# nygenome/lancet

Measured on AMD Instinct MI355X. Metric: assembled windows/sec (whole node), 600bp windows, self-tuning k, synthetic T/N, higher is better.
Workload: dtype u64; 1 GPU; chr22-scan proxy: 32768 windows/GPU x 600 bp, stride 100, 30x tumor / 30x normal, 2x150 bp, k=11..101, active-region-off; windows_per_gpu=32768, reads_per_gpu=5895305, records_rank0_contig=22477, slots_in_flight=4080, batches_in_flight=2, windows_first_graph_in_lds=32768, graphs_built_ahead=2147, graphs_taken_from_pool=2037, windows_rerun_worst_case_tier=0

## Files before the change

lancet_amd/csrc/kernels.h:

```cpp
#pragma once
#include "wave.h"
#include "layout.h"
#include "../../include/lancet_engine.h"

#ifndef LANCET_WG
#define LANCET_WG 64
#endif
#ifdef LANCET_FAT
#define LC_QLANES LC_FAT_LANES
#define LC_PF_G 6
#define LC_QSTAGE (3 * LC_FAT_LANES)
#else
#define LC_QLANES LANCET_WG
#define LC_QSTAGE LC_STAGE
#endif

enum {
  EV_PROCESS = 1, EV_REPEAT_REF, EV_NEAR_REF, EV_READS, EV_STATS, EV_MARKREF, EV_LOWCOV, EV_CLEANDEAD,
  EV_COMPRESS, EV_CC, EV_CCID, EV_CCEND, EV_TRIM, EV_AMBIG_SRC, EV_NOMATCH_SRC, EV_AMBIG_SNK, EV_NOMATCH_SNK,
  EV_CYCLE, EV_TIPS_ROUND, EV_TIPS_REMOVED, EV_LINKS, EV_LOOKREP, EV_MISSING, EV_SEARCH, EV_NEAR_QRY,
  EV_DFSLIMIT, EV_PATH, EV_TS, EV_PATH_END, EV_EKA_END, EV_FOUND, EV_END
};

struct WinShared {
// ... 4159 lines not shown
  for (int j = 0; j < 3; ++j) {
    if (r.nh[j] < t.hrmnN[j]) t.hrmnN[j] = r.nh[j];
    if (r.th[j] < t.hrmnT[j]) t.hrmnT[j] = r.th[j];
    t.hrsumN[j] = (uint16_t)(t.hrsumN[j] + r.nh[j]); t.hrsumT[j] = (uint16_t)(t.hrsumT[j] + r.th[j]);
  }
}
DEV void ref_hp_at(const Ctx &c, uint32_t pos, HPc &r) {
  for (int j = 0; j < 3; ++j) { r.nh[j] = r.th[j] = r.nq[j] = r.tq[j] = 0; }
  if (!LC_SREF(c).LR || (int)pos >= LC_SREF(c).reflen) return;
  const uint16_t *h = LC_CTX(c).W->refhp + 6 * pos;
  for (int j = 0; j < 3; ++j) { r.th[j] = h[j]; r.nh[j] = h[3 + j]; }
}
DEV void path_hp_at(const Ctx &c, int P, HPc &a) {
  for (int j = 0; j < 3; ++j) { a.nh[j] = a.th[j] = a.nq[j] = a.tq[j] = 0; }
  if (!LC_SREF(c).LR) return;
  uint32_t d = LC_CTX(c).W->pdesc[P];
  desc_hp(c, d, 0, a.nh, a.nq);
  desc_hp(c, d, 1, a.th, a.tq);
}
template <class T> DEV void ts_add_alt(T &t, const uint16_t *n4, const uint16_t *t4) { for (int q = 0; q < 4; ++q) { acc_push(t.aN[q], n4[q]); acc_push(t.aT[q], t4[q]); } }
template <class T> DEV void ts_add_ref(T &t, const uint16_t *n2, const uint16_t *t2) { for (int q = 0; q < 2; ++q) { acc_push(t.rN[q], n2[q]); acc_push(t.rT[q], t2[q]); } }

DEV void ref_cov_at(const Ctx &c, uint32_t pos, uint16_t *n2, uint16_t *t2) {
  if ((int)pos < LC_SREF(c).reflen) { const uint16_t *r = LC_CTX(c).W->refcov + 4 * pos; t2[0] = r[0]; t2[1] = r[1]; n2[0] = r[2]; n2[1] = r[3]; }
  else { n2[0] = n2[1] = t2[0] = t2[1] = 0; }
}
DEV void path_cov_at(const Ctx &c, int P, uint16_t *n4, uint16_t *t4) {
  uint32_t d = LC_CTX(c).W->pdesc[P];
  desc_cov(c, d, 0, &n4[0], &n4[1], &n4[2], &n4[3]);
  desc_cov(c, d, 1, &t4[0], &t4[1], &t4[2], &t4[3]);
}

DEV void bx_add_node(Ctx &c, uint32_t X, uint32_t nml, uint32_t *n) {
  LC_GLOBAL Work &W = *LC_CTX(c).W; LC_GLOBAL const DevBatch &B = *LC_CTX(c).B; LC_WS &S = LC_SREF(c);
  const uint32_t g0 = B.read_begin[S.w], refr = (uint32_t)(S.R - 1);
  LC_GLOBAL uint32_t *buf = W.bxbuf;
  for (uint32_t i = W.nocc[X]; i < W.nocc[X + 1]; ++i) {
    const uint32_t r = CS_READ(W_CSR(W)[i]);
    if (r == refr) continue;
    if (RI_NML(B.rinfo[g0 + r]) != nml) continue;
    const uint32_t bx = B.bx_rank[g0 + r];
    if (bx == 0xFFFFFFFFu) continue;
    uint32_t lo = 0, hi = *n;
    while (lo < hi) { uint32_t mid = (lo + hi) >> 1; if (buf[mid] < bx) lo = mid + 1; else hi = mid; }
    if (lo < *n && buf[lo] == bx) continue;
    if (*n >= LC_CTX(c).C->reads_cap) { OVF(c); return; }
    for (uint32_t j = *n; j > lo; --j) buf[j] = buf[j - 1];
    buf[lo] = bx; ++*n;
  }
}
DEVNI uint32_t kmer_lookup(Ctx &c, const uint8_t *codes, int *ori) {
  LC_GLOBAL Work &W = *LC_CTX(c).W; LC_WS &S = LC_SREF(c);
  const int K = S.K, NW = S.NW;
  unsigned long long fw[LC_NWMAX], rc[LC_NWMAX];
  for (int w = 0; w < LC_NWMAX; ++w) { fw[w] = 0; rc[w] = 0; }
  for (int i = 0; i < K; ++i) { key_push_fw(fw, NW, K, codes[i] & 3); key_push_rc(rc, NW, K, codes[i] & 3); }
  const unsigned long long *ck = key_less(fw, rc, NW) ? fw : rc;
  if (ori) *ori = ck == fw ? 0 : (key_less(rc, fw, NW) ? 1 : 2);
  const uint32_t mask = S.tmask;
  unsigned long long h = 0; uint32_t idx;
  if (NW == 1 && K <= 31) { h = ck[0] + 1ULL; idx = (uint32_t)mix64(h) & mask; }
  else {
    for (int w = 0; w < NW; ++w) h = mix64(h ^ (ck[w] + 0x9e3779b97f4a7c15ULL * (unsigned long long)(w + 1)));
    h &= ~(1ULL << 63);
    if (h == 0) h = 1;
    idx = (uint32_t)h & mask;
  }
  for (uint32_t probes = 0; probes <= mask; ++probes) {
    const unsigned long long cur = SL_TAG(W, idx);
    if (cur == 0) return LC_NIL;
    if (cur == h) {
      bool same = true;
      if (!(NW == 1 && K <= 31)) for (int w = 0; w < NW; ++w) if (W.slot_key[(size_t)idx * LC_NWMAX + w] != ck[w]) same = false;
      if (same) return SL_NODE(W, idx);
    }
    idx = (idx + 1) & mask;
  }
  return LC_NIL;
}
DEVNI void emit_variant_lr(Ctx &c, uint32_t vi, const TS &t, const uint16_t hp12[12], int plen) {
  LC_WS &S = LC_SREF(c); LC_GLOBAL Work &W = *LC_CTX(c).W; DevOut &O = *LC_CTX(c).OUT;
  lancet_variant_lr &l = O.variants_lr[vi];
  for (int q = 0; q < 12; ++q) l.hp[q] = hp12[q];
  l.reserved[0] = l.reserved[1] = 0;
  const int K = S.K;
  const uint32_t ro = W.occ_base[S.R - 1];
  for (int q = 0; q < 4; ++q) {
    const uint32_t nml = (q == 0 || q == 2) ? 1u : 0u;
    uint32_t n = 0;
    if (q < 2) {
      for (int i = (int)t.ref_pos - 1; i <= (int)t.ref_end_pos - 1; ++i) {
        if (i < 0 || i + K > S.seq_len) continue;
        const uint32_t rv = S.prebuilt ? W.lr_refnode[S.seq_t5 + i] : 0u;
        const uint32_t X = S.prebuilt ? (rv & 0x3FFFFFFFu) : (W.occ[ro + (uint32_t)(S.seq_t5 + i)] & 0x3FFFFFFFu);
        if (S.prebuilt ? (rv >> 31) != 0u : (W.gr[X].flags & NF_INMER) != 0u) bx_add_node(c, X, nml, &n);
      }
    } else {
      for (int i = (int)t.start_pos - 2; i <= (int)t.end_pos - 1; ++i) {
        if (i < 0 || i + K > plen) continue;
        const uint32_t X = kmer_lookup(c, W.pseq + i);
        if (X != LC_NIL) bx_add_node(c, X, nml, &n);
      }
    }
    const uint32_t off = dev_atomic_add(O.n_bx, n);
    if (off + n > LC_CTX(c).C->bx_cap) { OVF(c); l.bx_off[q] = 0; l.bx_len[q] = 0; continue; }
    l.bx_off[q] = off; l.bx_len[q] = n;
    for (uint32_t j = 0; j < n; ++j) O.bx_blob[off + j] = W.bxbuf[j];
  }
}

DEVNI void emit_variant(Ctx &c, const TS &t, const uint16_t cov[8], int strLen, const uint8_t *motif, int motifLen, bool hasStr,
                      const uint8_t *ra, const uint8_t *pa, const uint16_t hp12[12], int plen) {
  LC_WS &S = LC_SREF(c); DevOut &O = *LC_CTX(c).OUT;
  uint32_t vi = dev_atomic_add(O.n_variants, 1u);
  int rl = t.col1 - t.col0 + 1;
  char sbuf[80]; int sl = 0;
  if (hasStr) {
    char digs[12]; int nd = 0; int v = strLen; do { digs[nd++] = (char)('0' + v % 10); v /= 10; } while (v);
    while (nd) sbuf[sl++] = digs[--nd];
    for (int i = 0; i < motifLen; ++i) sbuf[sl++] = "ACGT"[motif[i]];
  }
  uint32_t need = (uint32_t)(2 * rl + sl);
  uint32_t bo = dev_atomic_add(O.n_blob, need);
  if (vi >= LC_CTX(c).C->var_cap || bo + need > LC_CTX(c).C->blob_cap) { OVF(c); return; }
  lancet_variant &v = O.variants[vi];
  v.window = S.w; v.seq_in_window = S.emit_seq++; v.chr_id = LC_CTX(c).B->chr_id[S.w]; v.pos = (int32_t)t.pos - 1;
  v.code = (uint8_t)t.code; v.prev_bp_ref = (uint8_t)t.prev_bp_ref; v.prev_bp_alt = (uint8_t)t.prev_bp_alt; v.reserved = 0;
  v.kmer = (uint16_t)S.K; for (int q = 0; q < 8; ++q) v.cov[q] = cov[q]; v.reserved2 = 0;
  v.ref_off = bo; v.ref_len = (uint32_t)rl; v.alt_off = bo + (uint32_t)rl; v.alt_len = (uint32_t)rl; v.str_off = bo + 2u * (uint32_t)rl; v.str_len = (uint32_t)sl;
  for (int i = 0; i < rl; ++i) { O.blob[bo + i] = (char)ra[t.col0 + i]; O.blob[bo + rl + i] = (char)pa[t.col0 + i]; }
  for (int i = 0; i < sl; ++i) O.blob[bo + 2 * rl + i] = sbuf[i];
  if (S.LR) emit_variant_lr(c, vi, t, hp12, plen);
}

DEVNI void walk_prepare(Ctx &c, int L) {
  LC_WS &S = LC_SREF(c); LC_GLOBAL Work &W = *LC_CTX(c).W;
  const int cap = (int)LC_CTX(c).C->max_w + (int)LC_CTX(c).C->path_cap + 2;
  LC_GLOBAL const uint8_t *ra = W.aln, *pa = W.aln + cap;
  LC_GLOBAL uint32_t *E1 = W.scratch, *E2 = W.scratch + (L + 1), *F = W.scratch + 2 * (L + 1), *cols = W.scratch + 3 * (L + 1);
  WG_LANE0 { S.wk[0] = S.wk[1] = S.wk[2] = S.wk[3] = 0; E1[L] = 0; E2[L] = 0; F[L] = 0; }
  WG_FOR(i, L) {
    const uint8_t r = ra[i], p = pa[i];
    E1[i] = r != '-'; E2[i] = p != '-'; F[i] = r != p;
    const int t = r == p ? 0 : (r == '-' ? 2 : (p == '-' ? 3 : 1));
    dev_atomic_add((LC_LDS uint32_t *)&S.wk[t], 1u);
  }
  WG_SYNC();
  wg_scan(E1, L + 1, S, S.part2);
  wg_scan(E2, L + 1, S, S.part2);
  wg_scan(F, L + 1, S, S.part2);
  WG_FOR(i, L) { if (F[i + 1] != F[i]) cols[F[i]] = (uint32_t)i; }
  WG_LANE0 { S.wk_n = (int)F[L]; }
}

DEVNI void process_path_walk(Ctx &c, int np, int plen, int L, int complete) {
  LC_WS &S = LC_SREF(c); LC_GLOBAL Work &W = *LC_CTX(c).W;
  const int K = S.K;
  const int cap = (int)LC_CTX(c).C->max_w + (int)LC_CTX(c).C->path_cap + 2;
  LC_GLOBAL const uint8_t *ra = W.aln, *pa = W.aln + cap;
  const int refstart = LC_CTX(c).B->ref_start[S.w];
  TS *ts = (TS *)(void *)W.tb;
  auto ts_at = [&](int idx) -> TS & { return ts[idx]; };
  int nts = 0;
  unsigned pos_in_ref = 0, pathpos = 0;
  char code = '?', prev_code = '?';
  const int match_bp = S.wk[0], snp_bp = S.wk[1], ins_bp = S.wk[2], del_bp = S.wk[3];
  LC_GLOBAL const uint32_t *E1 = W.scratch, *E2 = W.scratch + (L + 1), *cols = W.scratch + 3 * (L + 1);
  int pc_i = 0, pc_cur = 0;
  int last_col = -2;
  for (int ci = 0; ci < S.wk_n; ++ci) {
    const int i = (int)cols[ci];
    prev_code = (last_col == i - 1) ? code : '=';
    last_col = i;
    if (ra[i] == '-') code = '^'; else if (pa[i] == '-') code = 'v'; else code = 'x';
    pos_in_ref = E1[i];
    pathpos = E2[i] + (pa[i] != '-' ? 1u : 0u);
    uint32_t spanner = LC_NIL;
    for (; pc_i < np; ++pc_i) {
      const uint32_t nd = W.pnodes[pc_i];
      if (W.gr[nd].flags & NF_SPECIAL) continue;
      const int span = n_len(c, nd);
      if (pc_cur + span >= (int)pathpos) { spanner = nd; break; }
      pc_cur += span - K + 1;
    }
    if (spanner == LC_NIL) break;
    bool within_tumor = status_cnt_T(c, spanner);
    int P = (int)pathpos - 1;
    if (P < 0 || P >= plen) { OVF(c); return; }
    {
      uint16_t cn4[4], ct4[4], rn2[2], rt2[2];
      path_cov_at(c, P, cn4, ct4);
      ref_cov_at(c, pos_in_ref + (uint32_t)S.trim5, rn2, rt2);
      HPc ha, hr;
      path_hp_at(c, P, ha);
      ref_hp_at(c, pos_in_ref + (uint32_t)S.trim5, hr);
      unsigned rrpos = pos_in_ref + (unsigned)refstart + (unsigned)S.trim5;
      int pr = i - 1, pq = i - 1;
      while (pr >= 0 && ra[pr] != 'A' && ra[pr] != 'C' && ra[pr] != 'G' && ra[pr] != 'T') --pr;
      while (pq >= 0 && pa[pq] != 'A' && pa[pq] != 'C' && pa[pq] != 'G' && pa[pq] != 'T') --pq;
      if (pr < 0 || pq < 0) { OVF(c); return; }
      if (nts > 0 && prev_code != '=') {
        TS &t = ts_at(nts - 1);
        if (within_tumor) t.somatic = true;
        int reflen_before = t.col1 - t.col0 + 1;
        t.col1 = i; t.end_pos = (uint32_t)P; t.ref_end_pos = pos_in_ref;
        if (code == '^' && t.code == code && t.pos == rrpos) { ts_add_alt(t, cn4, ct4); ts_hp_add_alt(t, ha); }
        else if (code == 'v' && t.code == code && (t.pos + (unsigned)(reflen_before + 1)) == rrpos) { ts_add_ref(t, rn2, rt2); ts_hp_add_ref(t, hr); }
        else if (code == 'x' || t.code != code) { t.code = 'c'; ts_add_alt(t, cn4, ct4); ts_add_ref(t, rn2, rt2); ts_hp_add_alt(t, ha); ts_hp_add_ref(t, hr); }
      } else {
        if (nts >= LC_MAXTS) { OVF(c); return; }
        TS &t = ts_at(nts++);
        t.pos = rrpos; t.ref_pos = pos_in_ref; t.start_pos = (uint32_t)(P + 1); t.code = code; t.end_pos = (uint32_t)P; t.ref_end_pos = pos_in_ref;
        t.col0 = i; t.col1 = i; t.somatic = within_tumor; t.prev_bp_ref = (char)ra[pr]; t.prev_bp_alt = (char)pa[pq];
        for (int q = 0; q < 4; ++q) { acc_init(t.aN[q], cn4[q]); acc_init(t.aT[q], ct4[q]); }
        for (int q = 0; q < 2; ++q) { acc_init(t.rN[q], rn2[q]); acc_init(t.rT[q], rt2[q]); }
        ts_hp_init(t, ha, hr);
      }
    }
  }
  evt(c, EV_PATH, (uint32_t)complete, (uint32_t)S.tmp3, (uint32_t)match_bp, (uint32_t)snp_bp, (uint32_t)ins_bp, (uint32_t)del_bp);
  int ct_i = 0, ct_cur = 0, ct_last = -1;
  auto contig_at = [&](int pos) -> uint32_t {
    if (pos < ct_last) { ct_i = 0; ct_cur = 0; }
    ct_last = pos;
    for (; ct_i < np; ++ct_i) {
      const uint32_t nd = W.pnodes[ct_i];
      if (W.gr[nd].flags & NF_SPECIAL) continue;
      const int span = n_len(c, nd);
      if (ct_cur + span >= pos) return nd;
      ct_cur += span - K + 1;
    }
    return LC_NIL;
  };
  for (int ti = 0; ti < nts; ++ti) {
    TS &t = ts_at(ti);
    if (t.code != 'x') {
      for (int j = 0; j <= K; ++j) {
        unsigned idx1 = t.end_pos + (unsigned)j;
        if (idx1 < (unsigned)plen) {
          uint32_t sp = contig_at((int)idx1);
          if (sp == LC_NIL) break;
          if (status_cnt_T(c, sp)) t.somatic = true;
          uint16_t cn4[4], ct4[4];
          path_cov_at(c, (int)idx1, cn4, ct4);
          ts_add_alt(t, cn4, ct4);
          if (S.LR) { HPc ha; path_hp_at(c, (int)idx1, ha); ts_hp_add_alt(t, ha); }
        }
        unsigned idx2 = t.ref_end_pos + (unsigned)S.trim5 + (unsigned)j;
        uint16_t rn2[2], rt2[2];
        ref_cov_at(c, idx2, rn2, rt2);
        ts_add_ref(t, rn2, rt2);
        if (S.LR) { HPc hr; ref_hp_at(c, idx2, hr); ts_hp_add_ref(t, hr); }
      }
    }
    bool x = t.code == 'x';
    uint16_t RCNF = t.rN[0].mn, RCNR = t.rN[1].mn, RCTF = t.rT[0].mn, RCTR = t.rT[1].mn;
    uint16_t ACNF = x ? t.aN[2].mn : t.aN[0].mn, ACNR = x ? t.aN[3].mn : t.aN[1].mn;
    if (!x) { ACNF = t.aN[0].mnz; ACNR = t.aN[1].mnz; }
    uint16_t ACTF = x ? t.aT[2].mn : t.aT[0].mn, ACTR = x ? t.aT[3].mn : t.aT[1].mn;
    if (t.somatic) { RCNF = acc_mean(t.rN[0]); RCNR = acc_mean(t.rN[1]); RCTF = acc_mean(t.rT[0]); RCTR = acc_mean(t.rT[1]); ACNF = 0; ACNR = 0; }
    uint16_t cov[8] = {RCNF, RCNR, RCTF, RCTR, ACNF, ACNR, ACTF, ACTR};
    uint16_t hp12[12];
    {
      const uint32_t nref = t.rN[0].n;
      auto mean = [&](uint16_t sum) -> uint16_t { return nref > 0 ? (uint16_t)((float)sum / (float)nref) : (uint16_t)0; };
      uint16_t RN[3], RT[3], AN[3], AT[3];
      for (int j = 0; j < 3; ++j) {
        RN[j] = t.hrmnN[j]; RT[j] = t.hrmnT[j];
        AN[j] = x ? t.haqN[j] : t.hamnN[j]; AT[j] = x ? t.haqT[j] : t.hamnT[j];
        if (t.somatic) { RT[j] = mean(t.hrsumT[j]); RN[j] = mean(t.hrsumN[j]); AN[j] = 0; }
        if (!S.LR) { RN[j] = RT[j] = AN[j] = AT[j] = 0; }
      }
      const uint16_t v[12] = {RN[1], RN[2], RN[0], RT[1], RT[2], RT[0], AN[1], AN[2], AN[0], AT[1], AT[2], AT[0]};
      for (int q = 0; q < 12; ++q) hp12[q] = v[q];
    }
    if (LC_CTX(c).C->evt_cap) {
      evt(c, EV_TS, t.pos, (uint32_t)(t.col1 - t.col0 + 1), ((uint32_t)RCNF << 16) | RCNR, ((uint32_t)RCTF << 16) | RCTR,
          ((uint32_t)ACNF << 16) | ACNR, ((uint32_t)ACTF << 16) | ACTR, ((uint32_t)(uint8_t)t.prev_bp_ref << 8) | (uint8_t)t.prev_bp_alt);
      evt_bytes(c, ra + t.col0, (uint32_t)(t.col1 - t.col0 + 1));
      evt_bytes(c, pa + t.col0, (uint32_t)(t.col1 - t.col0 + 1));
      evt_bytes(c, (const uint8_t *)hp12, 24);
    }
    if (ACNF > 0 || ACNR > 0 || ACTF > 0 || ACTR > 0) {
      int LEN = 0, ml = 0; uint8_t motif[64];
      bool ans = find_tandems_local(c, W.pseq, plen, (int)t.start_pos, &LEN, motif, &ml);
      emit_variant(c, t, cov, LEN, motif, ml, ans, ra, pa, hp12, plen);
    }
  }
  evt(c, EV_PATH_END);
  for (int i = 0; i < np; ++i) ++W.gr[W.pnodes[i]].onref;
  if ((snp_bp + ins_bp + del_bp) == 0) ++S.tmp0; else if (snp_bp == 0) ++S.tmp1; else if ((ins_bp + del_bp) == 0) ++S.tmp2; else ++S.part[0];
}

DEV void walk_gather(Ctx &c, volatile LC_LDS uint32_t *rec, int pathpos, int P, uint32_t refpos, int plen, int np, LC_GLOBAL const uint32_t *pend, uint32_t w6, uint32_t w8, uint32_t code, bool lr = false) {
  LC_GLOBAL Work &W = *LC_CTX(c).W;
  uint32_t fl = 0;
  int lo = 0, hi = np;
  while (lo < hi) { const int mid = (lo + hi) >> 1; if ((int)(pend[2 * mid] & 0x7FFFFFFFu) >= pathpos) hi = mid; else lo = mid + 1; }
  while (lo < np && (pend[2 * lo] & 0x80000000u)) ++lo;
  if (lo >= np) fl |= 2u; else if (pend[2 * lo + 1] & 1u) fl |= 1u;
  uint16_t cn4[4] = {0, 0, 0, 0}, ct4[4] = {0, 0, 0, 0}, rn2[2], rt2[2];
  if (P < 0 || P >= plen) fl |= 4u; else path_cov_at(c, P, cn4, ct4);
  ref_cov_at(c, refpos, rn2, rt2);
  rec[0] = (uint32_t)cn4[0] | ((uint32_t)cn4[1] << 16); rec[1] = (uint32_t)cn4[2] | ((uint32_t)cn4[3] << 16);
  rec[2] = (uint32_t)ct4[0] | ((uint32_t)ct4[1] << 16); rec[3] = (uint32_t)ct4[2] | ((uint32_t)ct4[3] << 16);
  rec[4] = (uint32_t)rn2[0] | ((uint32_t)rn2[1] << 16); rec[5] = (uint32_t)rt2[0] | ((uint32_t)rt2[1] << 16);
// ... 178 lines not shown
          RN[j] = t.hrmnN[j]; RT[j] = t.hrmnT[j];
          AN[j] = x ? t.haqN[j] : t.hamnN[j]; AT[j] = x ? t.haqT[j] : t.hamnT[j];
          if (t.somatic) { RT[j] = mean(t.hrsumT[j]); RN[j] = mean(t.hrsumN[j]); AN[j] = 0; }
        }
        const uint16_t v[12] = {RN[1], RN[2], RN[0], RT[1], RT[2], RT[0], AN[1], AN[2], AN[0], AT[1], AT[2], AT[0]};
        for (int q = 0; q < 12; ++q) hp12[q] = v[q];
      }
      if (LC_CTX(c).C->evt_cap) {
        evt(c, EV_TS, t.pos, (uint32_t)(t.col1 - t.col0 + 1), ((uint32_t)RCNF << 16) | RCNR, ((uint32_t)RCTF << 16) | RCTR,
            ((uint32_t)ACNF << 16) | ACNR, ((uint32_t)ACTF << 16) | ACTR, ((uint32_t)(uint8_t)t.prev_bp_ref << 8) | (uint8_t)t.prev_bp_alt);
        evt_bytes(c, ra + t.col0, (uint32_t)(t.col1 - t.col0 + 1));
        evt_bytes(c, pa + t.col0, (uint32_t)(t.col1 - t.col0 + 1));
        evt_bytes(c, (const uint8_t *)hp12, 24);
      }
      if (ACNF > 0 || ACNR > 0 || ACTF > 0 || ACTR > 0) {
        int LEN = 0, ml = 0; uint8_t motif[64];
        bool ans = find_tandems_local(c, W.pseq, plen, (int)t.start_pos, &LEN, motif, &ml, stg, stg_lo, stg_hi);
        TS tc; tc.pos = t.pos; tc.ref_pos = t.ref_pos; tc.start_pos = t.start_pos; tc.end_pos = t.end_pos; tc.ref_end_pos = t.ref_end_pos; tc.col0 = t.col0; tc.col1 = t.col1;
        tc.code = t.code; tc.prev_bp_ref = t.prev_bp_ref; tc.prev_bp_alt = t.prev_bp_alt; tc.somatic = t.somatic;
        emit_variant(c, tc, cov, LEN, motif, ml, ans, ra, pa, hp12, plen);
      }
    }
    SUBPHASE(c, 4, 5);
  }
  SUBPHASE(c, 4, 7);
  WG_LANE0 { evt(c, EV_PATH_END); }
  WG_FOR(i, np) { dev_atomic_add(&W.gr[W.pnodes[i]].onref, 1u); }
  WG_LANE0 { const int snp_bp = S.wk[1], ins_bp = S.wk[2], del_bp = S.wk[3]; if ((snp_bp + ins_bp + del_bp) == 0) ++S.tmp0; else if (snp_bp == 0) ++S.tmp1; else if ((ins_bp + del_bp) == 0) ++S.tmp2; else ++S.part[0]; }
}

DEVNI void pcache_store(Ctx &c) {
  LC_WS &S = LC_SREF(c); LC_GLOBAL Work &W = *LC_CTX(c).W;
  LC_GLOBAL uint32_t *pc = W.mv;
  const uint32_t capw = 4u * LC_CTX(c).C->occ_cap;
  WG_LANE0 {
    const uint32_t n = (uint32_t)S.tmp2, pl = (uint32_t)S.tmp3, need = 4u + 2u * n + pl + (pl + 3u) / 4u;
    if (S.pc_top + need > capw) S.pc_ok = 0;
    else { pc[S.pc_top] = n; pc[S.pc_top + 1] = pl; pc[S.pc_top + 2] = (uint32_t)S.pc_bits; pc[S.pc_top + 3] = (uint32_t)S.pc_dfs; S.pc_base = S.pc_top; S.pc_top += need; ++S.pc_n; }
  }
  if (!wg_bcast(&S.pc_ok)) return;
  const uint32_t base = wg_bcastu(&S.pc_base), n = (uint32_t)wg_bcast(&S.tmp2), pl = (uint32_t)wg_bcast(&S.tmp3);
  WG_FOR(i, n) { pc[base + 4u + (uint32_t)i] = W.pnodes[i]; pc[base + 4u + n + (uint32_t)i] = W.pedges[i]; }
  WG_FOR(i, pl) { pc[base + 4u + 2u * n + (uint32_t)i] = W.pdesc[i]; }
  WG_FOR(i, (pl + 3u) / 4u) { pc[base + 4u + 2u * n + pl + (uint32_t)i] = ((LC_GLOBAL const uint32_t *)W.pseq)[i]; }
  WG_SYNC();
}
DEVNI int pcache_load(Ctx &c) {
  LC_WS &S = LC_SREF(c); LC_GLOBAL Work &W = *LC_CTX(c).W;
  LC_GLOBAL const uint32_t *pc = W.mv;
  const uint32_t base = wg_bcastu(&S.pc_base);
  const uint32_t n = pc[base], pl = pc[base + 1];
  WG_FOR(i, n) { W.pnodes[i] = pc[base + 4u + (uint32_t)i]; W.pedges[i] = pc[base + 4u + n + (uint32_t)i]; }
  WG_FOR(i, pl) { W.pdesc[i] = pc[base + 4u + 2u * n + (uint32_t)i]; }
  WG_FOR(i, (pl + 3u) / 4u) { ((LC_GLOBAL uint32_t *)W.pseq)[i] = pc[base + 4u + 2u * n + pl + (uint32_t)i]; }
  WG_SYNC();
  return (int)pl;
}
DEVNI bool repeats_in_graph_paths(Ctx &c) {
  LC_WS &S = LC_SREF(c); LC_GLOBAL Work &W = *LC_CTX(c).W;
  WG_LANE0 {
    evt(c, EV_LOOKREP);
    S.tmp0 = 0;
    if (S.source == LC_NIL || S.sink == LC_NIL) { evt(c, EV_MISSING); S.tmp0 = 1; }
    else evt(c, EV_SEARCH, (uint32_t)W.gr[S.source].comp);
    S.tmp1 = 0;
    S.pc_ok = 1; S.pc_n = 0; S.pc_top = 0; S.pc_end_dfs = 0;
  }
  while (wg_bcast(&S.tmp0) == 0) {
    SUBPHASE(c, 3, 2);
    const bool gcached = graph_cache_wg(c);
    WG_LANE0 {
      uint32_t best = gcached ? bfs_cached(c) : bfs(c);
      if (best == LC_NIL || S.overflow) { S.tmp0 = 1; S.pc_end_dfs = S.bfs_dfs; }
      else { S.tmp2 = path_unpack(c, best); S.pc_bits = (W.queue[best].bits & 2) ? 1 : 0; S.pc_dfs = S.bfs_dfs; }
    }
    if (wg_bcast(&S.tmp0) != 0) break;
    SUBPHASE(c, 3, 3);
    { const int pl = path_string_wg(c, wg_bcast(&S.tmp2)); WG_LANE0 { S.tmp3 = pl; if (S.overflow) S.tmp0 = 1; } }
    SUBPHASE(c, 3, 4);
    if (wg_bcast(&S.tmp0) != 0) break;
    {
      const int pl = wg_bcast(&S.tmp3);
      LC_GLOBAL const uint8_t *rs = LC_CTX(c).B->ref_codes + LC_CTX(c).B->ref_off[S.w] + S.seq_t5;
      const int rl = wg_uniform(S.seq_len), ml = pl < rl ? pl : rl;
      const bool tested = S.reflen - S.K > 0;
      WG_LANE0 { S.ps_hd = 0x7FFFFFFF; S.ps_tl = 0x7FFFFFFF; }
      WG_SYNC();
      if (tested) {
        WG_FOR(i, ml) {
          if (rs[i] != W.pseq[i]) dev_atomic_min((LC_LDS uint32_t *)&S.ps_hd, (uint32_t)i);
          if (rs[rl - 1 - i] != W.pseq[pl - 1 - i]) dev_atomic_min((LC_LDS uint32_t *)&S.ps_tl, (uint32_t)i);
        }
      }
      const int hd = wg_bcast(&S.ps_hd), tl = wg_bcast(&S.ps_tl);
      if (tested && pl == rl && hd == 0x7FFFFFFF) { WG_LANE0 { S.repE = 0; S.repM = 0; } }
      else if (!tested) repeat_scan_min(S.rs, W.pseq, pl, LC_CTX(c).P->max_mismatch, 0x7FFF, wg_uniform(S.K) + 1, &S.repE, &S.repM, nullptr, &S.rs_bad);
      else {
        const int a = hd < ml ? hd : ml;
        int sf = tl < ml ? tl : ml; if (a + sf > ml) sf = ml - a;
        const int b = pl - sf, K1 = wg_uniform(S.K) + 1;
        repeat_scan_min(S.rs, W.pseq, pl, LC_CTX(c).P->max_mismatch, 0x7FFF, K1, &S.repE, &S.repM, nullptr, &S.rs_bad, a - K1, b + K1);
      }
    }
    SUBPHASE(c, 3, 5);
    WG_LANE0 {
      if (S.tmp3 - S.K > 0 && S.repM >= S.K + 1) { evt(c, EV_NEAR_QRY, S.K); S.tmp0 = 2; }
      else {
        path_flag_edges(c, S.tmp2, 1u);
        for (int j = 1; j < S.tmp2; ++j) { if ((uint32_t)S.tmp1 < LC_CTX(c).C->node_cap) W.scratch[S.tmp1++] = W.pedges[j]; else { OVF(c); S.tmp0 = 1; } }
      }
    }
    SUBPHASE(c, 3, 6);
    if (wg_bcast(&S.tmp0) == 0 && wg_bcast(&S.pc_ok)) pcache_store(c);
  }
  SUBPHASE(c, 3, 10);
  WG_LANE0 {
    for (int j = 0; j < S.tmp1; ++j) { uint32_t owner = W.scratch[j] >> 4, ei = W.scratch[j] & 15u; W.gr[owner].edges[ei] &= ~(1u << 30); }
    if (S.tmp0 != 1 || S.overflow) S.pc_ok = 0;
  }
  return wg_bcast(&S.tmp0) == 2;
}

DEVNI void count_ref_path(Ctx &c) {
  LC_WS &S = LC_SREF(c); LC_GLOBAL Work &W = *LC_CTX(c).W;
  if (wg_bcastu(&S.source) == LC_NIL) return;
  if (wg_bcastu(&S.sink) != LC_NIL) {
    WG_LANE0 { evt(c, EV_SEARCH, (uint32_t)W.gr[S.source].comp); S.tmp0 = S.tmp1 = S.tmp2 = 0; S.part[0] = 0; S.part[1] = 0; S.part[2] = 0; S.part[3] = 0; S.pc_i = 0; S.pc_rd = 0; }
    const bool replay = wg_bcast(&S.pc_ok) != 0;
    while (wg_bcastu(&S.part[3]) == 0) {
      WG_LANE0 {
        if (replay) {
          if (S.pc_i < S.pc_n) {
            LC_GLOBAL const uint32_t *pc = W.mv + S.pc_rd;
            const uint32_t n = pc[0], pl = pc[1];
            if (pc[3]) evt(c, EV_DFSLIMIT);
            S.tmp3 = (int)pc[2];
            if (S.tmp3) ++S.part[2];
            ++S.part[1];
            S.part[4] = n;
            S.pc_base = S.pc_rd; S.pc_rd += 4u + 2u * n + pl + (pl + 3u) / 4u; ++S.pc_i;
          } else { if (S.pc_end_dfs) evt(c, EV_DFSLIMIT); S.part[3] = 1; }
        } else {
          uint32_t best = bfs(c);
          if (best == LC_NIL || S.overflow) S.part[3] = 1;
          else {
            S.tmp3 = (W.queue[best].bits & 2) ? 1 : 0;
            if (S.tmp3) ++S.part[2];
            ++S.part[1];
            S.part[4] = (uint32_t)path_unpack(c, best);
          }
        }
      }
      if (wg_bcastu(&S.part[3]) != 0) break;
      {
        const int m = replay ? pcache_load(c) : path_string_wg(c, (int)wg_bcastu(&S.part[4]));
        const int n = wg_bcast(&S.seq_len);
        LC_GLOBAL const uint8_t *rs = LC_CTX(c).B->ref_codes + LC_CTX(c).B->ref_off[S.w] + S.seq_t5;
        WG_LANE0 { S.ps_hd = 0; }
        if (n == m) { WG_FOR(i, n) { if (rs[i] != W.pseq[i]) dev_atomic_add((LC_LDS uint32_t *)&S.ps_hd, 1u); } }
        WG_SYNC();
        const int hd = (n == m) ? wg_uniform(S.ps_hd) : -1;
        const bool need_align = (hd == -1 || hd > 5);
        if (!need_align) {
          const int cap = (int)LC_CTX(c).C->max_w + (int)LC_CTX(c).C->path_cap + 2;
          WG_FOR(i, n) { W.aln[i] = "ACGTN"[rs[i]]; W.aln[cap + i] = "ACGT"[W.pseq[i]]; }
        }
        WG_LANE0 {
          S.part[5] = (uint32_t)m; S.part[6] = need_align ? 1u : 0u;
          if (!need_align) S.part[7] = (uint32_t)n;
          if (n > (int)LC_CTX(c).C->max_w || n < 1 || m < 1) OVF(c);
          if (S.overflow) S.part[3] = 1;
        }
      }
      if (wg_bcastu(&S.part[3]) != 0) break;
      if (wg_bcastu(&S.part[6])) {
        LC_GLOBAL const uint8_t *rs = LC_CTX(c).B->ref_codes + LC_CTX(c).B->ref_off[S.w] + S.seq_t5;
        const int pl = (int)wg_bcastu(&S.part[5]);
        PHASE(c, 12);
        if (!align_fill_band(c, rs, S.seq_len, W.pseq, pl)) align_fill(c, rs, S.seq_len, W.pseq, pl);
        PHASE(c, 13);
        { const int aL = align_traceback_wg(c, rs, S.seq_len, W.pseq, pl); WG_LANE0 { S.part[7] = (uint32_t)aL; } }
        WG_SYNC();
        align_traceback_fill(c, rs, W.pseq, (int)wg_bcastu(&S.part[7]));
      }
      PHASE(c, 14);
      SUBPHASE(c, 4, 2);
      walk_prepare(c, (int)wg_bcastu(&S.part[7]));
      SUBPHASE(c, 4, 14);
#ifdef LANCET_WAVE_EMU
      const bool old_walk = getenv("LANCET_OLD_WALK") != nullptr;
#else
      const bool old_walk = false;
#endif
#ifdef LANCET_LR_WALK_LANE0
      if (old_walk || wg_uniform(S.LR)) {
#else
      if (old_walk) {
#endif
        WG_LANE0 { if (!S.overflow) process_path_walk(c, (int)S.part[4], (int)S.part[5], (int)S.part[7], (int)S.part[1]); }
      } else if (!wg_bcast(&S.overflow)) {
        process_path_walk_wg(c, (int)wg_bcastu(&S.part[4]), (int)wg_bcastu(&S.part[5]), (int)wg_bcastu(&S.part[7]), (int)wg_bcastu(&S.part[1]));
      }
      WG_LANE0 {
        if (!S.overflow) path_flag_edges(c, (int)S.part[4], 1u);
        if (S.overflow) S.part[3] = 1;
      }
      PHASE(c, 11);
    }
    WG_LANE0 { evt(c, EV_EKA_END, (uint32_t)S.refcomp, S.part[1], S.part[2], (uint32_t)S.tmp0, (uint32_t)S.tmp2, (uint32_t)S.tmp1, S.part[0]); }
  }
  WG_LANE0 {
    if (LC_CTX(c).C->evt_cap) { uint32_t n = 0; for (uint32_t i = 0; i < S.M; ++i) if (W.gr[W.order[i]].onref) ++n; evt(c, EV_FOUND, n); }
  }
  WG_SYNC();
}

DEVNI void load_prebuilt_lr(Ctx &c, LC_GLOBAL const uint8_t *area) {
  LC_WS &S = LC_SREF(c); LC_GLOBAL Work &W = *LC_CTX(c).W;
  LC_GLOBAL const PreLayout &PL = LC_PL(c);
  LC_GLOBAL const PreHdr *H = (LC_GLOBAL const PreHdr *)(area + PRE_OFF_HDR);
  const uint32_t N = H->N, ncand = H->ncand, nsurv = H->nsurv, total = H->lr_total;
  const int K = S.K, NW = S.NW, reflen = S.reflen;
  LC_GLOBAL const uint32_t *lrnocc = (LC_GLOBAL const uint32_t *)(area + PRE_OFF_LRNOCC), *lrcsr = (LC_GLOBAL const uint32_t *)(area + PRE_OFF_LRCSR);
  LC_GLOBAL const uint32_t *occ_ref = (LC_GLOBAL const uint32_t *)(area + PRE_OFF_OCCREF);
  LC_GLOBAL const uint32_t *snode = (LC_GLOBAL const uint32_t *)(area + PRE_OFF_SNODE), *sid = (LC_GLOBAL const uint32_t *)(area + PRE_OFF_SID);
  LC_GLOBAL const unsigned long long *skey = (LC_GLOBAL const unsigned long long *)(area + PRE_OFF_SKEY);
  LC_GLOBAL const uint8_t *surv = (LC_GLOBAL const uint8_t *)(area + PRE_OFF_SURV);
  const int nrefk = reflen - K > 0 ? reflen - K + 1 : 0;
  const int t5 = wg_bcast(&S.seq_t5), L = wg_bcast(&S.seq_len);
  PHASE(c, 2);
  WG_LANE0 { W.qv = W.qv_own; }
  WG_FOR(r, S.R) {
    uint32_t rinfo, bw, gw; int tlen; bool isref;
    read_geom(c, r, &rinfo, &bw, &gw, &tlen, &isref);
    W.rd[4 * r] = rinfo; W.rd[4 * r + 1] = bw; W.rd[4 * r + 2] = gw; W.rd[4 * r + 3] = 0;
  }
  WG_FOR(n, N + 1) { W.nocc[n] = lrnocc[n]; }
  WG_FOR(i, total) { const uint32_t v = lrcsr[i]; W_CSR(W)[i] = CS_MAKE(v & 0xFFFFu, (v >> 16) & 0x3FFu, (v >> 26) & 1u, (v >> 27) & 3u); }
  WG_FOR(i, (N + 31u) / 32u) { W.bitmap[i] = 0; W.bitpre[i] = 0; }
  WG_SYNC();
  WG_FOR(i, nrefk) {
    const uint32_t n = occ_ref[i] & 0x3FFFFFFFu & ~PB_GONE;
    dev_atomic_or(&W.bitmap[n >> 5], 1u << (n & 31u));
    if (i >= t5 && i - t5 < L - K) dev_atomic_or(&W.bitpre[n >> 5], 1u << (n & 31u));
  }
  WG_LANE0 { S.tmp2 = 0; }
  WG_SYNC();
  WG_FOR(i, nrefk) {
    const uint32_t n = occ_ref[i] & 0x3FFFFFFFu & ~PB_GONE;
    W.lr_refnode[i] = n | (((ld2(&W.bitpre[n >> 5]) >> (n & 31u)) & 1u) << 31);
  }
  PHASE(c, 4);
  WG_FOR(n, N) {
    const bool onr = ((ld2(&W.bitmap[(uint32_t)n >> 5]) >> ((uint32_t)n & 31u)) & 1u) != 0;
    if (!surv[n] && !onr) continue;
    const uint32_t lo = lrnocc[n], hi = lrnocc[n + 1];
    if (hi - lo >= LR_COOP_MIN && hi - lo <= LR_COOP_MAX && lo < (1u << 24)) {
      const uint32_t at = dev_atomic_add((LC_LDS uint32_t *)&S.tmp2, 1u);
      W.scratch[2 * (size_t)at] = (uint32_t)n; W.scratch[2 * (size_t)at + 1] = lo | ((hi - lo) << 24);
    } else {
      uint32_t lrv[10] = {0, 0, 0, 0, 0, 0, 0, 0, 0, 0};
      if (hi > lo) lr_node_replay(c, lo, hi, lrv);
      LC_GLOBAL NodeGr &G = W.gr[n];
      for (int q = 0; q < 4; ++q) G.kc[q] = (uint16_t)lrv[q];
      for (int q = 0; q < 6; ++q) W.khp[6 * (size_t)n + q] = (uint16_t)lrv[4 + q];
      G.mincov = (int)(uint16_t)lrv[0] + (int)(uint16_t)lrv[1] + (int)(uint16_t)lrv[2] + (int)(uint16_t)lrv[3];
    }
  }
  WG_SYNC();
  PHASE(c, 5);
  lr_replay_batches(c, (uint32_t)wg_bcast(&S.tmp2));
  PHASE(c, 6);
  WG_FOR(si, nsurv) {
    const uint32_t n = sid[si];
    W.pnodes[si] = n; W.pedges[si] = lrnocc[n]; W.ht_bucket[si] = lrnocc[n + 1] - lrnocc[n]; W.ht_start[si] = W.gr[n].nqv;
  }
  WG_SYNC();
  if (nsurv) build_qcounts(c, nsurv);
  if (wg_bcast(&S.overflow)) return;
  PHASE(c, 3);
  WG_FOR(j, reflen) { for (int q = 0; q < 4; ++q) W.refcov[4 * j + q] = 0; for (int q = 0; q < 6; ++q) W.refhp[6 * j + q] = 0; }
  WG_SYNC();
  WG_FOR(i, reflen - K > 0 ? reflen - K : 0) {
    const uint32_t rv = W.lr_refnode[i], X = rv & 0x3FFFFFFFu;
    uint16_t v[4] = {0, 0, 0, 0}, h[6] = {0, 0, 0, 0, 0, 0};
    if (rv >> 31) {
      for (int q = 0; q < 4; ++q) v[q] = W.gr[X].kc[q];
      for (int q = 0; q < 6; ++q) h[q] = W.khp[6 * (size_t)X + q];
    }
    if (i == 0) { for (int j = 0; j < K; ++j) { for (int q = 0; q < 4; ++q) W.refcov[4 * j + q] = v[q]; for (int q = 0; q < 6; ++q) W.refhp[6 * j + q] = h[q]; } }
    else { for (int q = 0; q < 4; ++q) W.refcov[4 * (i + K - 1) + q] = v[q]; for (int q = 0; q < 6; ++q) W.refhp[6 * (i + K - 1) + q] = h[q]; }
  }
  WG_LANE0 { uint32_t tcap = 1024; while (tcap < 2u * nsurv + 2u && tcap < LC_CTX(c).C->table_cap) tcap <<= 1; S.tmask = tcap - 1u; S.tfull = 0; }
  const uint32_t mask = wg_bcastu(&S.tmask);
  WG_FOR(i, mask + 1u) { lc_u4 z; z.x = 0; z.y = 0; z.z = LC_NIL; z.w = 0; *(lc_u4 *)(W.slots + 4 * (size_t)i) = z; }
  WG_SYNC_FENCE();
  WG_FOR(ci, ncand) {
    const uint32_t n = snode[ci];
    if (n == LC_NIL) continue;
    unsigned long long ck[LC_NWMAX];
    for (int w = 0; w < LC_NWMAX; ++w) ck[w] = w < NW ? skey[(size_t)ci * PL.kw + (uint32_t)w] : 0ULL;
    unsigned long long h = 0; uint32_t idx;
    if (NW == 1 && K <= 31) { h = ck[0] + 1ULL; idx = (uint32_t)mix64(h) & mask; }
    else {
      for (int w = 0; w < NW; ++w) h = mix64(h ^ (ck[w] + 0x9e3779b97f4a7c15ULL * (unsigned long long)(w + 1)));
      h &= ~(1ULL << 63);
      if (h == 0) h = 1;
      idx = (uint32_t)h & mask;
    }
    for (uint32_t probes = 0; probes <= mask; ++probes) {
      const unsigned long long old = dev_atomic_cas64(&SL_TAG(W, idx), 0ULL, h);
      if (old == 0ULL) { SL_NODE(W, idx) = n; if (!(NW == 1 && K <= 31)) for (int w = 0; w < NW; ++w) W.slot_key[(size_t)idx * LC_NWMAX + w] = ck[w]; break; }
      idx = (idx + 1) & mask;
    }
  }
  WG_SYNC_FENCE();
}

DEVNI bool load_prebuilt(Ctx &c, int k) {
  LC_WS &S = LC_SREF(c); LC_GLOBAL Work &W = *LC_CTX(c).W;
  LC_GLOBAL const uint8_t *pre = LC_CTX(c).OUT->pre;
  if (!pre) return false;
  LC_GLOBAL const PreLayout &PL = LC_PL(c);
  LC_GLOBAL const uint8_t *area = pre + (size_t)S.w * PRE_STRIDE;
  LC_GLOBAL const PreHdr *H = (LC_GLOBAL const PreHdr *)(area + PRE_OFF_HDR);
  for (int hop = 0; hop < 16 && H->status == PB_BUILT && H->K < k && H->next != 0u && LC_CTX(c).OUT->pre_pool; ++hop) {
    area = LC_CTX(c).OUT->pre_pool + (size_t)(H->next - 1u) * PRE_STRIDE;
    H = (LC_GLOBAL const PreHdr *)(area + PRE_OFF_HDR);
  }
  WG_LANE0 { S.tmp1 = (H->status == PB_BUILT && H->K == k && H->N <= LC_CTX(c).C->node_cap && (size_t)H->ncand * (size_t)k <= (size_t)LC_CTX(c).C->qv_cap &&
                       H->ncand <= LC_CTX(c).C->surv_cap && (size_t)H->ncand * (size_t)k <= (size_t)LC_CTX(c).C->seq_cap) ? 1 : 0;
             if (S.LR && !(H->lr == 1u && H->have_order == 1u && H->lr_total <= LC_CTX(c).C->occ_cap)) S.tmp1 = 0; }
  if (!wg_bcast(&S.tmp1)) return false;
  const uint32_t N = H->N, ncand = H->ncand, nsurv = H->nsurv;
  const int K = k;
  WG_LANE0 {
    if (S.n_builds > 0 && LC_CTX(c).OUT->n_ahead_used) dev_atomic_add(LC_CTX(c).OUT->n_ahead_used, 1u);
    S.N = N; S.N_last = N; S.O = H->O; S.totalreadbp = (int)H->totalreadbp; S.n_kmers += (unsigned long long)H->n_kmers; ++S.n_builds;
    if (N > S.max_nodes) S.max_nodes = N;
    S.sum_nodes += N;
    S.nspecial = 0; S.qv_top = ncand; S.seq_top = ncand * (uint32_t)K; S.tmask = 0; S.tfull = 0; S.prebuilt = 1;
    S.pre_edges = H->edges_total; S.pre_refn = H->refn;
    W.occ_base[S.R - 1] = 0;
    S.pre_order = H->have_order == 1u ? 1 : 0;
    if (S.pre_order) {
      S.M = nsurv; S.ht_bc = H->ht_bc; S.ht_elt = nsurv; S.ht_next_resize = H->ht_next_resize; S.ht_head = LC_NIL;
      S.numcomp = (int)H->numcomp; S.refcomp = (int)H->refcomp;
    }
  }
  const bool pre_order = H->have_order == 1u;
  LC_GLOBAL const unsigned long long *nhash = (LC_GLOBAL const unsigned long long *)(area + PRE_OFF_NHASH);
  LC_GLOBAL const uint8_t *surv = (LC_GLOBAL const uint8_t *)(area + PRE_OFF_SURV);
  LC_GLOBAL const uint32_t *snode = (LC_GLOBAL const uint32_t *)(area + PRE_OFF_SNODE), *sid = (LC_GLOBAL const uint32_t *)(area + PRE_OFF_SID);
  LC_GLOBAL const unsigned long long *skey = (LC_GLOBAL const unsigned long long *)(area + PRE_OFF_SKEY);
// ... 504 lines not shown
```

Baseline: 878,000 windows/s.

## Fast-path perfect and near-reference paths in the variant walk, skipping scans

When the assembled path matches the reference exactly (Hamming distance 0), the walk now skips building the alignment strings, the three prefix scans and the full variant walk. It only emits the path events and marks path nodes as on-reference. For paths with a few mismatches (at most 5), mismatch positions are recorded during the Hamming count, and a lane-0 insertion sort builds the column list in place of the workgroup scans. This targets the common case of reads that agree with the reference, at the cost of extra code paths whose sparse E1/E2 arrays must stay equivalent to what the full walk expects.

```diff
diff --git a/lancet_amd/csrc/kernels.h b/lancet_amd/csrc/kernels.h
--- a/lancet_amd/csrc/kernels.h
+++ b/lancet_amd/csrc/kernels.h
@@ -4335,6 +4335,29 @@
   WG_FOR(i, L) { if (F[i + 1] != F[i]) cols[F[i]] = (uint32_t)i; }
   WG_LANE0 { S.wk_n = (int)F[L]; }
 }
+#define LC_HD_MAX 5
+DEVNI void walk_prepare_unaligned(Ctx &c, int L, int hd) {
+  LC_WS &S = LC_SREF(c); LC_GLOBAL Work &W = *LC_CTX(c).W;
+  LC_GLOBAL uint32_t *E1 = W.scratch, *E2 = W.scratch + (L + 1), *cols = W.scratch + 3 * (L + 1);
+  WG_LANE0 {
+    for (int a = 1; a < hd; ++a) {
+      const uint32_t v = S.part2[a]; int b = a;
+      for (; b > 0 && S.part2[b - 1] > v; --b) S.part2[b] = S.part2[b - 1];
+      S.part2[b] = v;
+    }
+    for (int a = 0; a < hd; ++a) { const uint32_t i = S.part2[a]; cols[a] = i; E1[i] = i; E2[i] = i; }
+    S.wk[0] = L - hd; S.wk[1] = hd; S.wk[2] = 0; S.wk[3] = 0; S.wk_n = hd;
+  }
+}
+DEVNI void process_path_perfect_wg(Ctx &c, int np, int n, int complete) {
+  LC_WS &S = LC_SREF(c); LC_GLOBAL Work &W = *LC_CTX(c).W;
+  WG_LANE0 {
+    evt(c, EV_PATH, (uint32_t)complete, (uint32_t)S.tmp3, (uint32_t)n, 0u, 0u, 0u);
+    evt(c, EV_PATH_END);
+    ++S.tmp0;
+  }
+  WG_FOR(i, np) { dev_atomic_add(&W.gr[W.pnodes[i]].onref, 1u); }
+}
 
 DEVNI void process_path_walk(Ctx &c, int np, int plen, int L, int complete) {
   LC_WS &S = LC_SREF(c); LC_GLOBAL Work &W = *LC_CTX(c).W;
@@ -4819,16 +4842,28 @@
         }
       }
       if (wg_bcastu(&S.part[3]) != 0) break;
+#ifdef LANCET_WAVE_EMU
+      const bool old_walk = getenv("LANCET_OLD_WALK") != nullptr;
+#elif defined(LANCET_LR_WALK_LANE0)
+      const bool old_walk = wg_uniform(S.LR) != 0;
+#else
+      const bool old_walk = false;
+#endif
+      int hd = -1;
       {
         const int m = replay ? pcache_load(c) : path_string_wg(c, (int)wg_bcastu(&S.part[4]));
         const int n = wg_bcast(&S.seq_len);
         LC_GLOBAL const uint8_t *rs = LC_CTX(c).B->ref_codes + LC_CTX(c).B->ref_off[S.w] + S.seq_t5;
         WG_LANE0 { S.ps_hd = 0; }
-        if (n == m) { WG_FOR(i, n) { if (rs[i] != W.pseq[i]) dev_atomic_add((LC_LDS uint32_t *)&S.ps_hd, 1u); } }
+        if (n == m) {
+          WG_FOR(i, n) {
+            if (rs[i] != W.pseq[i]) { const uint32_t q = dev_atomic_add((LC_LDS uint32_t *)&S.ps_hd, 1u); if (q < (uint32_t)LC_HD_MAX) S.part2[q] = (uint32_t)i; }
+          }
+        }
         WG_SYNC();
-        const int hd = (n == m) ? wg_uniform(S.ps_hd) : -1;
-        const bool need_align = (hd == -1 || hd > 5);
-        if (!need_align) {
+        hd = (n == m) ? wg_uniform(S.ps_hd) : -1;
+        const bool need_align = (hd == -1 || hd > LC_HD_MAX);
+        if (!need_align && (hd > 0 || old_walk)) {
           const int cap = (int)LC_CTX(c).C->max_w + (int)LC_CTX(c).C->path_cap + 2;
           WG_FOR(i, n) { W.aln[i] = "ACGTN"[rs[i]]; W.aln[cap + i] = "ACGT"[W.pseq[i]]; }
         }
@@ -4851,22 +4886,19 @@
         align_traceback_fill(c, rs, W.pseq, (int)wg_bcastu(&S.part[7]));
       }
       PHASE(c, 14);
-      SUBPHASE(c, 4, 2);
-      walk_prepare(c, (int)wg_bcastu(&S.part[7]));
-      SUBPHASE(c, 4, 14);
-#ifdef LANCET_WAVE_EMU
-      const bool old_walk = getenv("LANCET_OLD_WALK") != nullptr;
-#else
-      const bool old_walk = false;
-#endif
-#ifdef LANCET_LR_WALK_LANE0
-      if (old_walk || wg_uniform(S.LR)) {
-#else
-      if (old_walk) {
-#endif
-        WG_LANE0 { if (!S.overflow) process_path_walk(c, (int)S.part[4], (int)S.part[5], (int)S.part[7], (int)S.part[1]); }
-      } else if (!wg_bcast(&S.overflow)) {
-        process_path_walk_wg(c, (int)wg_bcastu(&S.part[4]), (int)wg_bcastu(&S.part[5]), (int)wg_bcastu(&S.part[7]), (int)wg_bcastu(&S.part[1]));
+      if (hd == 0 && !old_walk) {
+        SUBPHASE(c, 4, 7);
+        if (!wg_bcast(&S.overflow)) process_path_perfect_wg(c, (int)wg_bcastu(&S.part[4]), (int)wg_bcastu(&S.part[7]), (int)wg_bcastu(&S.part[1]));
+      } else {
+        SUBPHASE(c, 4, 2);
+        if (hd > 0 && hd <= LC_HD_MAX && !old_walk) walk_prepare_unaligned(c, (int)wg_bcastu(&S.part[7]), hd);
+        else walk_prepare(c, (int)wg_bcastu(&S.part[7]));
+        SUBPHASE(c, 4, 14);
+        if (old_walk) {
+          WG_LANE0 { if (!S.overflow) process_path_walk(c, (int)S.part[4], (int)S.part[5], (int)S.part[7], (int)S.part[1]); }
+        } else if (!wg_bcast(&S.overflow)) {
+          process_path_walk_wg(c, (int)wg_bcastu(&S.part[4]), (int)wg_bcastu(&S.part[5]), (int)wg_bcastu(&S.part[7]), (int)wg_bcastu(&S.part[1]));
+        }
       }
       WG_LANE0 {
         if (!S.overflow) path_flag_edges(c, (int)S.part[4], 1u);
```

Measured after the change: 892,100 windows/s, median of 6. 1.6% higher.
